# rewaifu/resselt

Measured on AMD Instinct MI355X. Metric: output megapixels/sec, RealESRGAN-x4plus 1080p→4K, 1/2/4/8 MI355X, higher is better.
Workload: dtype fp16; 1 GPU; RealESRGAN-x4plus (RRDBNet nf64 nb23 gc32 x4), 1x3x1080x1920 fp32 frame per GPU -> 1x3x4320x7680, residual-dense-block convolutions (92 % of the MACs) in ONE fp16 product on hi planes, conv_first / upsampling / HR / last convolutions in three bf16 products on split planes, trunk convolution in three fp16 products; f32 accumulate, synthetic uniform(+-1/sqrt(fan_in)) weights; precision=auto -> mixed, io=fp32 [N,C,H,W] tensors in and out, tile_parallel=single tile

## Files before the change

resselt_amd/csrc/conv_ring.h:

```cpp
#pragma once
#include <hip/hip_runtime.h>
#include <stdint.h>

#include "conv_common.h"
#include "conv_kernel.h"

namespace rsa {

#ifdef RSA_RING_DEBUG
static __device__ unsigned int g_ring_dbg;
#define RING_DBG(bit) (dbg & (bit))
#else
#define RING_DBG(bit) false
#endif

static __device__ unsigned int g_ring_aborts;

static unsigned int ring_aborts_this_unit() {
  unsigned int v = 0;
  const unsigned int zero = 0;
  if (hipMemcpyFromSymbol(&v, HIP_SYMBOL(g_ring_aborts), sizeof(v)) != hipSuccess) return 0x10000000u;
  if (v != 0 && hipMemcpyToSymbol(HIP_SYMBOL(g_ring_aborts), &zero, sizeof(zero)) != hipSuccess) return 0x10000000u;
  return v;
}

typedef const __attribute__((address_space(1))) char* gcptr;

#ifndef RSA_RING_INFL1
#define RSA_RING_INFL1 2
#endif
#ifndef RSA_RING_WD1
#define RSA_RING_WD1 3
#endif
#ifndef RSA_RING_WDX
#define RSA_RING_WDX 4
#endif
#ifndef RSA_RING_DEPTH1
#define RSA_RING_DEPTH1 4
#endif

template <int PROD, int WL = 0>
struct RingGeoP {
  static constexpr int TH = 16, TW = 32, IH = 18, IW = 34;
  static constexpr int PS = 624;
  static constexpr int HALF = 2 * PS;
  static constexpr int NHL = PROD == 3 ? 2 : 1;
  static constexpr int SLOT = NHL * HALF;
  static constexpr int NSLOT = (PROD == 3 || WL) ? 4 : 8;
  static constexpr int DMA_IT = (HALF + 63) / 64;
  static constexpr int DPF = NHL * DMA_IT;
  static constexpr int INFL = (PROD == 3 || WL) ? 1 : RSA_RING_INFL1;
  static constexpr int WL_FRAGS = WL ? 45 : 0;
  static constexpr int BAND = 4;
  static constexpr int FLAG_UNITS = 5;
};
using RingGeo = RingGeoP<3>;

__device__ __forceinline__ void ring_tile_coords(int t, int tiles_x, int tiles_y, int& n, int& ty, int& tx) {
  const int tiles_img = tiles_x * tiles_y;
  n = t / tiles_img;
  const int r = t - n * tiles_img;
  const int band = r / (RingGeo::BAND * tiles_x);
  const int rr = r - band * RingGeo::BAND * tiles_x;
  const int rows = min(RingGeo::BAND, tiles_y - band * RingGeo::BAND);
  tx = rr / rows;
  ty = band * RingGeo::BAND + (rr - tx * rows);
}

__device__ __forceinline__ uint32_t lds_ld(const uint32_t* p) { return __hip_atomic_load(p, __ATOMIC_RELAXED, __HIP_MEMORY_SCOPE_WORKGROUP); }

__device__ __forceinline__ void ring_wait_slow(const uint32_t* flag, uint32_t need, uint32_t* abort_word, const RingAux& aux) {
  const int limit = __builtin_amdgcn_readfirstlane(aux.spin_limit);
  for (int spin = 0; spin < limit; ++spin) {
    __builtin_amdgcn_s_sleep(1);
    if (__builtin_amdgcn_readfirstlane(lds_ld(flag)) >= need) return;
    if ((spin & 63) == 63 && __builtin_amdgcn_readfirstlane(lds_ld(abort_word)) != 0) return;
  }
  __hip_atomic_store(abort_word, 1u, __ATOMIC_RELAXED, __HIP_MEMORY_SCOPE_WORKGROUP);
  if ((threadIdx.x & 63) == 0) {
    atomicAdd(&g_ring_aborts, 1u);
    if (aux.fail_word != nullptr) __hip_atomic_fetch_add(aux.fail_word, 1u, __ATOMIC_RELAXED, __HIP_MEMORY_SCOPE_SYSTEM);
  }
}
__device__ __forceinline__ void ring_wait(const uint32_t* flag, uint32_t need, uint32_t* abort_word, const RingAux& aux) {
  if (__builtin_expect(__builtin_amdgcn_readfirstlane(lds_ld(flag)) < need, 0)) ring_wait_slow(flag, need, abort_word, aux);
}

__device__ __forceinline__ gcptr uniform_ptr(gcptr q) {
  const uint64_t v = (uint64_t)q;
  const uint32_t lo = __builtin_amdgcn_readfirstlane((uint32_t)v), hi = __builtin_amdgcn_readfirstlane((uint32_t)(v >> 32));
  return (gcptr)(((uint64_t)hi << 32) | lo);
}

__device__ __forceinline__ void dma16_s(uint32_t lds_addr, uint32_t voff, gcptr sbase) {
  asm volatile("s_mov_b32 m0, %0\n\ts_nop 0\n\tglobal_load_lds_dwordx4 %1, %2" ::"s"(lds_addr), "v"(voff), "s"(sbase) : "memory");
}
__device__ __forceinline__ void dma16_v(uint32_t lds_addr, gcptr vaddr) {
  asm volatile("s_mov_b32 m0, %0\n\ts_nop 0\n\tglobal_load_lds_dwordx4 %1, off" ::"s"(lds_addr), "v"(vaddr) : "memory");
}

#ifndef RSA_C5_EPI
#define RSA_C5_EPI 1
#endif
#ifdef RSA_C5_STAMPS
static __device__ unsigned long long g_c5_stamps[256 * 8 * 8];
#define C5_ST_ARG , st
#else
#define C5_ST_ARG
#endif
template <int SHAPE, int UP, int OUTK, int HM = 0, int FMT = 0, int PROD = 3, int XRES = 0, int XAC = 0, int XR2 = -1>
__global__ __launch_bounds__((8 + (SHAPE == 2 ? 2 : 1)) * 64, 3) void conv_ring(const rsa_conv_params p, const RingAux aux) {
  static_assert(XR2 == -1 || XRES == 4 || XRES == 5, "XR2: the coded conv5 kernels only");
  static_assert((XRES != 1 && XRES != 4 && XRES != 5) || (SHAPE == 1 && PROD == 1 && HM == 0 && UP == 0 && OUTK == 0), "XRES 1 / 4 / 5: conv5 of a residual dense block only");
  static_assert(XRES != 2 || (PROD == 1 && FMT == RSA_PF_F16 && OUTK == 0), "XRES 2: one fp16 product, hi-only plane output");
  static_assert(XRES != 3 || (SHAPE == 3 && PROD == 1 && FMT == RSA_PF_F16 && HM == 1 && UP == 0 && OUTK == 0), "XRES 3: the 48-channel SPAN-family layers");
  static_assert(XRES != 6 || (SHAPE == 2 && OUTK == 1 && UP == 0), "XRES 6: final stores with at most 16 output channels");
  static_assert(XRES != 7 || (SHAPE != 2 && UP == 0 && OUTK == 0), "XRES 7: plane output, one tile stream");
  constexpr bool WL = XRES == 3;
  constexpr bool XR = XRES == 1 || XRES == 4 || XRES == 5;
  using R = RingGeoP<PROD, WL>;
  constexpr int STREAMS = SHAPE == 2 ? 2 : 1;
  constexpr int TH = R::TH, TW = R::TW, IH = R::IH, IW = R::IW, PS = R::PS, HALF = R::HALF, SLOT = R::SLOT, NSLOT = R::NSLOT;
  constexpr int NHL = R::NHL, INFL = R::INFL;
  constexpr int WBASE = NSLOT * SLOT + R::FLAG_UNITS;
  constexpr int NCT = SHAPE == 2 ? 2 : (SHAPE == 1 ? 4 : 3);
  constexpr int CTW = SHAPE == 3 ? 3 : 2;
  constexpr int NPT = SHAPE == 3 ? 4 : 8;
  constexpr int CTU = XRES == 6 ? 1 : CTW;
  constexpr int RPW = NPT / 2;
  constexpr int NCONS = (STREAMS == 2) ? 4 : 8;
  constexpr int SPS = NSLOT / STREAMS;

  __shared__ uint4 s_ring[NSLOT * SLOT + R::FLAG_UNITS + R::WL_FRAGS * 64];
  uint32_t* const flags = (uint32_t*)&s_ring[NSLOT * SLOT];
  uint32_t* const f_full = flags;
  uint32_t* const f_free = flags + 8;
  uint32_t* const f_abort = flags + 16;

  const int tid = threadIdx.x;
  const int lane = tid & 63;
  const int wave = __builtin_amdgcn_readfirstlane(tid >> 6);

  const int tiles_x = (p.W + TW - 1) / TW;
  const int tiles_y = (p.H + TH - 1) / TH;
  const int num_tiles = tiles_x * tiles_y * p.batch;
  const int nhalf = p.cin_planes >> 1;
  const int nq = HM ? nhalf : (nhalf >> 1);
  const int ct_total = (p.cout + 15) >> 4;

  const int NWG = (int)gridDim.x;
  const int tile0 = (NWG % 8 == 0) ? ((int)blockIdx.x % 8) * (NWG / 8) + (int)blockIdx.x / 8 : (int)blockIdx.x;
  if (tile0 >= num_tiles) return;
  const int ntw = (num_tiles - tile0 + NWG - 1) / NWG;

  if (tid < 4 * R::FLAG_UNITS) flags[tid] = 0;
  if (WL) {
    const int wunits = nq * 5 * ct_total * 64;
    for (int i = tid; i < wunits; i += (int)blockDim.x) s_ring[WBASE + i] = ((const uint4*)p.w_packed)[i];
  }
  __syncthreads();
#ifdef RSA_RING_DEBUG
  const unsigned dbg = __builtin_amdgcn_readfirstlane(g_ring_dbg);
#endif

  if (wave >= 8) {
    __builtin_amdgcn_s_setprio(3);
    const int g = wave - 8;
    const int inW = UP ? (p.W >> 1) : p.W;
    uint32_t lc[R::DMA_IT];
    uint32_t smap[R::DMA_IT];
#pragma unroll
    for (int it = 0; it < R::DMA_IT; ++it) {
      const int u = it * 64 + lane;
      const int pl = (u / PS) & 1;
      const int r = u % PS;
      int py = r / IW, px = r - (r / IW) * IW;
      if (r >= IH * IW) py = 0, px = 0;
      smap[it] = (uint32_t)(pl << 16 | py << 8 | px);
      const int sy = UP ? ((py + 1) >> 1) : py;
      const int sx = UP ? ((px + 1) >> 1) : px;
      lc[it] = (uint32_t)(((int64_t)pl * p.in_plane_stride + (int64_t)sy * inW + sx) * 16);
    }
    const uint32_t ring_lds = (uint32_t)(uintptr_t)(__attribute__((address_space(3))) void*)s_ring;
    int k = 0;
    int pend_slot[INFL];
    uint32_t pend_val[INFL];
#pragma unroll
    for (int i = 0; i < INFL; ++i) pend_slot[i] = -1, pend_val[i] = 0;
    auto publish_all = [&]() {
      asm volatile("s_waitcnt vmcnt(0)" ::: "memory");
#pragma unroll
      for (int i = 0; i < INFL; ++i) {
        if (pend_slot[i] >= 0) __hip_atomic_store(&f_full[pend_slot[i]], pend_val[i], __ATOMIC_RELAXED, __HIP_MEMORY_SCOPE_WORKGROUP);
        pend_slot[i] = -1;
      }
    };
    for (int j = (STREAMS == 2 ? g : 0); j < ntw; j += STREAMS) {
      int n, ty, tx;
      ring_tile_coords(p.tile_order ? num_tiles - 1 - (tile0 + j * NWG) : tile0 + j * NWG, tiles_x, tiles_y, n, ty, tx);
      const int y0 = ty * TH - 1, x0 = tx * TW - 1;
      const bool interior = y0 >= 0 && x0 >= 0 && y0 + IH <= p.H && x0 + IW <= p.W;
      const int64_t tile_unit = (int64_t)n * p.in_batch_stride + (int64_t)(UP ? ty * (TH / 2) - 1 : y0) * inW + (UP ? tx * (TW / 2) - 1 : x0);
      for (int h = 0; h < nhalf; ++h, ++k) {
        const int slot = (STREAMS == 2) ? SPS * g + (k & (SPS - 1)) : (k & (NSLOT - 1));
        const uint32_t use = (uint32_t)(k / SPS);
        if (__builtin_amdgcn_readfirstlane(lds_ld(&f_free[slot])) < NCONS * use) {
          bool any = false;
#pragma unroll
          for (int i = 0; i < INFL; ++i) any = any || pend_slot[i] >= 0;
          if (any) publish_all();
          ring_wait(&f_free[slot], NCONS * use, f_abort, aux);
        }
        const int hh = XR ? 2 * (nq - 1 - (h >> 1)) + (h & 1) : h;
        const int64_t half_unit = tile_unit + (int64_t)(2 * hh) * p.in_plane_stride;
        gcptr bh = uniform_ptr((gcptr)p.in_hi + half_unit * 16);
        gcptr bl = uniform_ptr((gcptr)p.in_lo + half_unit * 16);
        const uint32_t dst = __builtin_amdgcn_readfirstlane(ring_lds + (uint32_t)slot * (SLOT * 16));
        if (RING_DBG(1)) {
        } else if (interior) {
#pragma unroll
          for (int it = 0; it < R::DMA_IT; ++it) {
            if (it == R::DMA_IT - 1 && lane >= 32) continue;
            dma16_s(dst + it * 1024, lc[it], bh);
            if (PROD == 3) dma16_s(dst + HALF * 16 + it * 1024, lc[it], bl);
          }
        } else {
#pragma unroll
          for (int it = 0; it < R::DMA_IT; ++it) {
            if (it == R::DMA_IT - 1 && lane >= 32) continue;
            const uint32_t m = smap[it];
            const int pl = (int)(m >> 16);
            int iy = y0 + (int)((m >> 8) & 255u), ix = x0 + (int)(m & 255u);
            const bool ok = (uint32_t)iy < (uint32_t)p.H && (uint32_t)ix < (uint32_t)p.W;
            if (UP) {
              iy >>= 1;
              ix >>= 1;
            }
            const int64_t off = ((int64_t)n * p.in_batch_stride + (int64_t)(2 * hh + pl) * p.in_plane_stride + (int64_t)iy * inW + ix) * 16;
            gcptr sh = ok ? (gcptr)p.in_hi + off : (gcptr)&g_zero_unit[0];
            dma16_v(dst + it * 1024, sh);
            if (PROD == 3) {
              gcptr sl = ok ? (gcptr)p.in_lo + off : (gcptr)&g_zero_unit[0];
              dma16_v(dst + HALF * 16 + it * 1024, sl);
            }
          }
        }
        if (pend_slot[0] >= 0) {
          asm volatile("s_waitcnt vmcnt(%0)" ::"n"(INFL * R::DPF) : "memory");
          __hip_atomic_store(&f_full[pend_slot[0]], pend_val[0], __ATOMIC_RELAXED, __HIP_MEMORY_SCOPE_WORKGROUP);
        }
#pragma unroll
        for (int i = 0; i + 1 < INFL; ++i) pend_slot[i] = pend_slot[i + 1], pend_val[i] = pend_val[i + 1];
        pend_slot[INFL - 1] = slot;
        pend_val[INFL - 1] = use + 1;
      }
    }
    publish_all();
    return;
  }

  const int g = (STREAMS == 2) ? (wave >> 2) : 0;
  const int wct = (SHAPE == 1) ? (wave >> 2) : 0;
  const int wpx = (SHAPE == 3) ? wave : (wave & 3);
  const int li = lane & 15;
  const int lg = lane >> 4;
  const int hsel = lg >> 1;

  constexpr int KSU = HM ? 5 : 9;
  constexpr int WD = (PROD == 3 || WL) ? 1 : ((XRES && XRES != 7) ? RSA_RING_WDX : RSA_RING_WD1);
  const int nks = nq * KSU;
  const __amdgpu_buffer_rsrc_t rw = __builtin_amdgcn_make_buffer_rsrc((void*)p.w_packed, 0, (uint32_t)((int64_t)nks * ct_total * NHL * 64 * 16), 0x00020000);
  uint32_t woff[CTW];
#pragma unroll
  for (int c = 0; c < CTW; ++c) {
    const int ctg = wct * CTW + c;
    woff[c] = (ctg < ct_total) ? (uint32_t)((ctg * NHL * 64 + lane) * 16) : 0xFFFFFFFFu;
  }
  const uint32_t wstep = (uint32_t)ct_total * NHL * 64 * 16;
  bf16x8 wq[WD + 1][CTW][NHL];
  auto load_w = [&](int s) {
#pragma unroll
    for (int c = 0; c < CTU; ++c)
#pragma unroll
      for (int hl = 0; hl < NHL; ++hl) {
        if (RING_DBG(4)) continue;
        if (WL) {
          wq[WD][c][hl] = *(const bf16x8*)&s_ring[WBASE + (s * ct_total + wct * CTW + c) * 64 + lane];
          continue;
        }
        const u32x4 v = __builtin_amdgcn_raw_buffer_load_b128(rw, woff[c], (uint32_t)s * wstep + (uint32_t)hl * 1024u, 0);
        wq[WD][c][hl] = __builtin_bit_cast(bf16x8, v);
      }
  };
  auto shift_w = [&]() {
#pragma unroll
    for (int d = 0; d < WD; ++d)
#pragma unroll
      for (int c = 0; c < CTU; ++c)
#pragma unroll
        for (int hl = 0; hl < NHL; ++hl) wq[d][c][hl] = wq[d + 1][c][hl];
  };

  f32x4 acc[NPT][CTW];
#pragma unroll
  for (int pt = 0; pt < NPT; ++pt)
#pragma unroll
    for (int ct = 0; ct < CTW; ++ct) acc[pt][ct] = (f32x4){0.f, 0.f, 0.f, 0.f};

  const int lane_u = (lg & 1) * PS + (wpx * RPW) * IW + li;
  int uA1, uA2, uB1, uB2, uS;

#ifndef RSA_RING_STAGGER
#define RSA_RING_STAGGER 0
#endif
#ifndef RSA_RING_STAGGER_SLEEP
#define RSA_RING_STAGGER_SLEEP 100
#endif
#ifndef RSA_RING_PRIO_HI
#define RSA_RING_PRIO_HI 0
#endif
  if (RSA_RING_PRIO_HI && wave >= 4) __builtin_amdgcn_s_setprio(RSA_RING_PRIO_HI);
  if (RSA_RING_STAGGER) {
    if (STREAMS == 2 ? g == 1 : wave >= 4)
      for (int d = 0; d < nq * RSA_RING_STAGGER; ++d) __builtin_amdgcn_s_sleep(RSA_RING_STAGGER_SLEEP);
  }

  auto wmap = [&](int c, int koff) -> int {
    int cc = c + koff / KSU;
    if (cc >= nq) cc -= nq;
    return (XR ? nq - 1 - cc : cc) * KSU + koff % KSU;
  };
#pragma unroll
  for (int d = 0; d < WD; ++d) {
    load_w(d < nks ? wmap(0, d) : wmap(0, 0));
    if (d + 1 < WD) {
#pragma unroll
      for (int e = 1; e < WD; ++e)
#pragma unroll
        for (int c = 0; c < CTW; ++c)
#pragma unroll
          for (int hl = 0; hl < NHL; ++hl) wq[e][c][hl] = wq[e + 1][c][hl];
    }
  }
  uint32_t kc = 0;
  auto slot_of = [&](uint32_t k) -> int { return (STREAMS == 2) ? SPS * g + (int)(k & (SPS - 1)) : (int)(k & (NSLOT - 1)); };
  auto use_of = [&](uint32_t k) -> uint32_t { return k / SPS; };
  uint32_t xslots = 0;
#ifdef RSA_C5_STAMPS
  unsigned long long st[8] = {0, 0, 0, 0, 0, 0, 0, 0};
  const unsigned long long t_begin = C5_TIME();
#endif
  for (int j = (STREAMS == 2 ? g : 0); j < ntw; j += STREAMS) {
    for (int c = 0; c < nq; ++c) {
      const int sA = slot_of(kc), sB = HM ? sA : slot_of(kc + 1);
      const uint32_t needA = use_of(kc) + 1, needB = use_of(kc + 1) + 1;
      if (XR) {
        if (c == nq - 2) xslots = (uint32_t)sA << 8 | (uint32_t)sB << 12;
        if (c == nq - 1) xslots |= (uint32_t)sA | (uint32_t)sB << 4;
      }
      {
        const int bA = sA * SLOT + lane_u, bB = sB * SLOT + lane_u;
        uA1 = bA + hsel;
        uA2 = bA + 2 + hsel * IW;
        uB1 = bB + hsel;
        uB2 = bB + 2 + hsel * IW;
        uS = (hsel ? bB : bA) + 2 * IW + 2;
      }
#ifdef RSA_C5_STAMPS
      const unsigned long long twA = C5_TIME();
#endif
      ring_wait(&f_full[sA], needA, f_abort, aux);
#ifdef RSA_C5_STAMPS
      st[1] += C5_TIME() - twA;
#endif
      __builtin_amdgcn_sched_barrier(0);
      asm volatile("" ::: "memory");

      constexpr int NSTEP = KSU * NPT;
      constexpr int DEPTH = PROD == 3 ? 2 : RSA_RING_DEPTH1;
      bf16x8 rh[DEPTH + 1], rl[PROD == 3 ? DEPTH + 1 : 1];
      auto frag = [&](int i) -> int {
        const int ks = i / NPT, pt = i % NPT;
        const int ptoff = (pt >> 1) * IW + (pt & 1) * 16;
        switch (ks) {
          case 0: return uA1 + ptoff;
          case 1: return uA1 + IW + ptoff;
          case 2: return uA1 + 2 * IW + ptoff;
          case 3: return uA2 + ptoff;
          case 4: return uS + ptoff;
          case 5: return uB1 + ptoff;
          case 6: return uB1 + IW + ptoff;
          case 7: return uB1 + 2 * IW + ptoff;
          default: return uB2 + ptoff;
        }
      };
#pragma unroll
      for (int i = 0; i < DEPTH; ++i) {
        rh[i] = *(const bf16x8*)&s_ring[frag(i)];
        if (PROD == 3) rl[i] = *(const bf16x8*)&s_ring[HALF + frag(i)];
      }
      auto step = [&](int i) {
        const int ks = i / NPT, sp = i % NPT;
        if (sp == 0) {
          shift_w();
          load_w(wmap(c, ks + WD));
          if (ks == 5) {
            asm volatile("" ::: "memory");
            if (lane == 0 && !(XR && c >= nq - 2)) __hip_atomic_fetch_add(&f_free[sA], 1u, __ATOMIC_RELAXED, __HIP_MEMORY_SCOPE_WORKGROUP);
          }
          __builtin_amdgcn_sched_barrier(0);
        }
        if (i + DEPTH < NSTEP && !RING_DBG(16)) {
          const int u = frag(i + DEPTH);
          rh[(i + DEPTH) % (DEPTH + 1)] = *(const bf16x8*)&s_ring[u];
          if (PROD == 3) rl[(i + DEPTH) % (DEPTH + 1)] = *(const bf16x8*)&s_ring[HALF + u];
        }
        if (!RING_DBG(2))
#pragma unroll
        for (int pr = 0; pr < PROD; ++pr)
#pragma unroll
          for (int ct = 0; ct < CTU; ++ct) {
            const bf16x8 wf = (PROD == 3 && pr == 0) ? wq[0][ct][NHL - 1] : wq[0][ct][0];
            const bf16x8 bf = (PROD == 3 && pr == 1) ? rl[PROD == 3 ? i % (DEPTH + 1) : 0] : rh[i % (DEPTH + 1)];
            acc[sp][ct] = mfma16<FMT>(wf, bf, acc[sp][ct]);
          }
        if (i + DEPTH < NSTEP) __builtin_amdgcn_sched_group_barrier(0x100, NHL, 0);
        __builtin_amdgcn_sched_group_barrier(0x008, PROD * CTU, 0);
        __builtin_amdgcn_sched_barrier(0);
      };
      if (HM) {
#pragma unroll
        for (int i = 0; i < NSTEP; ++i) step(i);
        asm volatile("" ::: "memory");
        if (lane == 0) __hip_atomic_fetch_add(&f_free[sA], 1u, __ATOMIC_RELAXED, __HIP_MEMORY_SCOPE_WORKGROUP);
        kc += 1;
      } else {
        constexpr int FIRST_B = 4 * NPT - DEPTH;
#pragma unroll
        for (int i = 0; i < FIRST_B; ++i) step(i);
#ifdef RSA_C5_STAMPS
        const unsigned long long twB = C5_TIME();
#endif
        ring_wait(&f_full[sB], needB, f_abort, aux);
#ifdef RSA_C5_STAMPS
        st[1] += C5_TIME() - twB;
#endif
        __builtin_amdgcn_sched_barrier(0);
        asm volatile("" ::: "memory");
#pragma unroll
        for (int i = FIRST_B; i < NSTEP; ++i) step(i);
        asm volatile("" ::: "memory");
        if (lane == 0 && !(XR && c >= nq - 2)) __hip_atomic_fetch_add(&f_free[sB], 1u, __ATOMIC_RELAXED, __HIP_MEMORY_SCOPE_WORKGROUP);
        kc += 2;
      }
    }
    {
      int n, ty, tx;
      ring_tile_coords(p.tile_order ? num_tiles - 1 - (tile0 + j * NWG) : tile0 + j * NWG, tiles_x, tiles_y, n, ty, tx);
      if (XRES == 2) {
        if (!RING_DBG(8)) epilogue_impl<NCT, CTW, NPT, 0, AC_LINEAR, 1, RSA_PF_F16>(p, acc, n, ty * TH, tx * TW, 0, wct, wpx, li, lg);
      } else if (XRES == 3) {
        if (!RING_DBG(8)) epilogue_impl<NCT, CTW, NPT, 0, XAC, 4, RSA_PF_F16>(p, acc, n, ty * TH, tx * TW, 0, wct, wpx, li, lg);
      } else if constexpr (XRES == 7) {
        if (!RING_DBG(8)) epilogue_impl<NCT, CTW, NPT, 0, AC_LINEAR, 5>(p, acc, n, ty * TH, tx * TW, 0, wct, wpx, li, lg);
      } else if (XR) {
#ifdef RSA_C5_STAMPS
        const unsigned long long te = C5_TIME();
#endif
        if (RING_DBG(8)) {
        } else if constexpr (XR2 >= 0) {
          epilogue_c5<XR2, XRES == 4 ? 1 : 2>(p, acc, n, ty * TH, tx * TW, wct, wpx, li, lg, s_ring, xslots, SLOT, PS, IW C5_ST_ARG);
        } else {
          if (p.res2_hi != nullptr)
            epilogue_impl<NCT, CTW, NPT, 0, AC_LINEAR, 3, RSA_PF_F16, 1, XRES == 4 ? 1 : (XRES == 5 ? 2 : 0)>(p, acc, n, ty * TH, tx * TW, 0, wct, wpx, li, lg, s_ring, xslots, SLOT, PS, IW C5_ST_ARG);
          else
            epilogue_impl<NCT, CTW, NPT, 0, AC_LINEAR, 2, RSA_PF_F16, 1, XRES == 4 ? 1 : (XRES == 5 ? 2 : 0)>(p, acc, n, ty * TH, tx * TW, 0, wct, wpx, li, lg, s_ring, xslots, SLOT, PS, IW C5_ST_ARG);
        }
#ifdef RSA_C5_STAMPS
        st[3] += C5_TIME() - te;
        st[4] += 1;
#endif
        asm volatile("s_waitcnt lgkmcnt(0)" ::: "memory");
        if (lane == 0) {
#pragma unroll
          for (int q = 0; q < 4; ++q) __hip_atomic_fetch_add(&f_free[(xslots >> (4 * q)) & 15u], 1u, __ATOMIC_RELAXED, __HIP_MEMORY_SCOPE_WORKGROUP);
        }
      } else if (!RING_DBG(8)) {
        epilogue<NCT, CTW, NPT, OUTK>(p, acc, n, ty * TH, tx * TW, 0, wct, wpx, li, lg);
      }
    }
#pragma unroll
    for (int pt = 0; pt < NPT; ++pt)
#pragma unroll
      for (int ct = 0; ct < CTW; ++ct) acc[pt][ct] = (f32x4){0.f, 0.f, 0.f, 0.f};
  }
#ifdef RSA_C5_STAMPS
  st[0] = C5_TIME() - t_begin;
  if (XR && lane == 0 && blockIdx.x < 256)
    for (int i = 0; i < 8; ++i) g_c5_stamps[((int)blockIdx.x * 8 + wave) * 8 + i] = st[i];
#endif
}

template <int SHAPE, int UP, int OUTK, int HM = 0, int FMT = 0, int PROD = 3, int XRES = 0, int XAC = 0, int XR2 = -1>
static int launch_ring(const rsa_conv_params& p, hipStream_t stream) {
  if constexpr ((XRES == 4 || XRES == 5) && XR2 == -1 && RSA_C5_EPI) {
    if (c5_epilogue_fits(p))
      return p.res2_hi != nullptr ? launch_ring<SHAPE, UP, OUTK, HM, FMT, PROD, XRES, XAC, 1>(p, stream) : launch_ring<SHAPE, UP, OUTK, HM, FMT, PROD, XRES, XAC, 0>(p, stream);
  }
  constexpr int STREAMS = SHAPE == 2 ? 2 : 1;
  using R = RingGeoP<PROD>;
  const int tiles_x = (p.W + R::TW - 1) / R::TW;
  const int tiles_y = (p.H + R::TH - 1) / R::TH;
  const int64_t num_tiles = (int64_t)tiles_x * tiles_y * p.batch;
  if (num_tiles > 0x3fffffff) return RSA_E_UNSUPPORTED;
  static const int cus = [] {
    int dev = 0;
    hipDeviceProp_t prop;
    if (hipGetDevice(&dev) != hipSuccess || hipGetDeviceProperties(&prop, dev) != hipSuccess) return 256;
    return prop.multiProcessorCount;
  }();
  int gx = cus;
  if (gx > num_tiles) gx = (int)num_tiles;
  hipLaunchKernelGGL((conv_ring<SHAPE, UP, OUTK, HM, FMT, PROD, XRES, XAC, XR2>), dim3((unsigned)gx, 1, 1), dim3((8 + STREAMS) * 64), 0, stream, p, ring_aux());
  return (int)hipGetLastError();
}

}
```

resselt_amd/csrc/conv_ring_pair.h:

```cpp
#pragma once
#include <type_traits>

#include "conv_ring.h"

namespace rsa {

struct PairParams {
  int32_t batch, H, W;
  int32_t nqa;
  const void* in_hi;
  int64_t in_plane_stride, in_batch_stride;
  const void* wa;
  const void* wb;
  const float* bias_a;
  const float* bias_b;
  float slope_a, slope_b;
  void* outa_hi;
  int64_t outa_unit0;
  int64_t outa_plane_stride, outa_batch_stride;
  void* outb_hi;
  int64_t outb_unit0;
  int64_t outb_plane_stride, outb_batch_stride;
  int32_t tile_order;
};

#ifndef RSA_PAIR_INFL
#define RSA_PAIR_INFL 1
#endif
#ifndef RSA_PAIR_WD
#define RSA_PAIR_WD 3
#endif
#ifndef RSA_PAIR_DEPTH
#define RSA_PAIR_DEPTH 3
#endif
#ifndef RSA_PAIR_PRIO_B
#define RSA_PAIR_PRIO_B 1
#endif
#ifndef RSA_PAIR_PRIO_A
#define RSA_PAIR_PRIO_A 0
#endif

#ifdef RSA_PAIR_STAMPS
static __device__ unsigned long long g_pair_stamps[256 * 9 * 8];
#define PSTAMP() __builtin_amdgcn_s_memtime()
#define PST_ADD(slot, t0) st[slot] += PSTAMP() - (t0)
#else
#define PSTAMP() 0ull
#define PST_ADD(slot, t0) (void)(t0)
#endif

struct PairGeo {
  static constexpr int TH = 16, TWO = 30;
  static constexpr int AH = 18, AW = 32;
  static constexpr int IH = 20, IW = 34;
  static constexpr int PS = 688;
  static constexpr int SLOT = 2 * PS;
  static constexpr int NSLOT = 5;
  static constexpr int DMA_IT = (SLOT + 63) / 64;
  static constexpr int INFL = RSA_PAIR_INFL;
  static constexpr int PSB = AH * AW;
  static constexpr int XB0 = NSLOT * SLOT;
  static constexpr int XB_UNITS = 4 * PSB + 16;
  static constexpr int FLAG_UNITS = 4;
  static constexpr int LDS_UNITS = XB0 + XB_UNITS + FLAG_UNITS;
  static_assert(SLOT % 64 == 32, "the last LDS-DMA instruction of a fill covers 32 units");
  static_assert(INFL * DMA_IT <= 63, "vmcnt");
  static_assert(LDS_UNITS * 16 <= 160 * 1024, "LDS");
};

__device__ __forceinline__ uint32_t pack_f16(float a, float b) {
  const f16x2 h = {(_Float16)a, (_Float16)b};
  return __builtin_bit_cast(uint32_t, h);
}

__device__ __forceinline__ uint4 pair_unit_f16(const f32x4 a, const f32x4 b, const f32x4 bias, float slope) {
  float va[4], vb[4];
#pragma unroll
  for (int r = 0; r < 4; ++r) {
    va[r] = a[r] + bias[r];
    vb[r] = b[r] + bias[r];
    va[r] = fmaxf(va[r], va[r] * slope);
    vb[r] = fmaxf(vb[r], vb[r] * slope);
  }
  const uint32_t a0 = pack_f16(va[0], va[1]), a1 = pack_f16(va[2], va[3]);
  const uint32_t b0 = pack_f16(vb[0], vb[1]), b1 = pack_f16(vb[2], vb[3]);
  const u32x2 h0 = __builtin_amdgcn_permlane16_swap(a0, b0, false, false);
  const u32x2 h1 = __builtin_amdgcn_permlane16_swap(a1, b1, false, false);
  return make_uint4(h0.x, h1.x, h0.y, h1.y);
}

template <int ROLE>
__device__ __forceinline__ void pair_consumer(const PairParams& p, const RingAux& aux, uint4* s_ring, uint32_t* flags, int wave, int lane, int tile0, int ntw,
                                              int NWG, int tiles_x, int tiles_y, int num_tiles) {
  using G = PairGeo;
  constexpr int IW = G::IW, PS = G::PS, SLOT = G::SLOT, NSLOT = G::NSLOT, AW = G::AW, PSB = G::PSB, XB0 = G::XB0;
  constexpr int CTW = 2, KSU = 9;
  constexpr int WD = RSA_PAIR_WD, DEPTH = RSA_PAIR_DEPTH;
  constexpr bool roleB = ROLE == 1;
  constexpr int NPT = roleB ? 8 : 9;
  uint32_t* const f_full = flags;
  uint32_t* const f_free = flags + 5;
  uint32_t* const f_abort = flags + 10;
  uint32_t* const f_xfull = flags + 11;
  uint32_t* const f_xfree = flags + 12;
  const int nqa = p.nqa;
#ifdef RSA_RING_DEBUG
  const unsigned dbg = __builtin_amdgcn_readfirstlane(g_ring_dbg);
#endif
  if (roleB && RSA_PAIR_PRIO_B) __builtin_amdgcn_s_setprio(RSA_PAIR_PRIO_B);
  if (!roleB && RSA_PAIR_PRIO_A) __builtin_amdgcn_s_setprio(RSA_PAIR_PRIO_A);
  const int r4 = wave & 3;
  const int li = lane & 15;
  const int lg = lane >> 4;
  const int hsel = lg >> 1;

  const int nunits = roleB ? nqa + 1 : nqa;
  const int nks = nunits * KSU;
  const __amdgpu_buffer_rsrc_t rw = __builtin_amdgcn_make_buffer_rsrc((void*)(roleB ? p.wb : p.wa), 0, (uint32_t)(nks * CTW * 64 * 16), 0x00020000);
  uint32_t woff[CTW];
#pragma unroll
  for (int c = 0; c < CTW; ++c) woff[c] = (uint32_t)((c * 64 + lane) * 16);
  constexpr uint32_t wstep = CTW * 64 * 16;
  bf16x8 wq[WD + 1][CTW];
  auto load_w = [&](int s) {
#pragma unroll
    for (int c = 0; c < CTW; ++c) {
      if (RING_DBG(4)) continue;
      const u32x4 v = __builtin_amdgcn_raw_buffer_load_b128(rw, woff[c], (uint32_t)s * wstep, 0);
      wq[WD][c] = __builtin_bit_cast(bf16x8, v);
    }
  };
  auto shift_w = [&]() {
#pragma unroll
    for (int d = 0; d < WD; ++d)
#pragma unroll
      for (int c = 0; c < CTW; ++c) wq[d][c] = wq[d + 1][c];
  };
  auto wmap = [&](int c, int koff) -> int {
    int cc = c + koff / KSU;
    if (cc >= nunits) cc -= nunits;
    return cc * KSU + koff % KSU;
  };
#pragma unroll
  for (int d = 0; d < WD; ++d) {
    load_w(d < nks ? wmap(0, d) : wmap(0, 0));
    if (d + 1 < WD) {
#pragma unroll
      for (int e = 1; e < WD; ++e)
#pragma unroll
        for (int c = 0; c < CTW; ++c) wq[e][c] = wq[e + 1][c];
    }
  }

  f32x4 acc[NPT][CTW];
#pragma unroll
  for (int pt = 0; pt < NPT; ++pt)
#pragma unroll
    for (int ct = 0; ct < CTW; ++ct) acc[pt][ct] = (f32x4){0.f, 0.f, 0.f, 0.f};

  const int lane_u = (lg & 1) * PS + (4 * r4 + (roleB ? 1 : 0)) * IW + li + (roleB ? 1 : 0);
  const int extra_u = __builtin_amdgcn_readfirstlane((16 + (r4 >> 1) - 4 * r4) * IW + (r4 & 1) * 16);
  const int lane_ub = XB0 + (lg & 1) * PSB + (4 * r4) * AW + li;

  int slot = 0;
  uint32_t use = 0;
  uint32_t tcount = 0;
#ifdef RSA_PAIR_STAMPS
  unsigned long long st[8] = {0, 0, 0, 0, 0, 0, 0, 0};
  const unsigned long long t_begin = PSTAMP();
#endif

  auto run_unit = [&](auto rs_tag, auto ring_tag, int c, int bA, int bB, int sA, int sB, uint32_t needA, uint32_t needB) {
    constexpr int RS = decltype(rs_tag)::value;
    constexpr bool RING = decltype(ring_tag)::value;
    constexpr int NSTEP = KSU * NPT;
    const int uA1 = bA + hsel, uA2 = bA + 2 + hsel * RS, uB1 = bB + hsel, uB2 = bB + 2 + hsel * RS;
    const int uS = (hsel ? bB : bA) + 2 * RS + 2;
    {
      const unsigned long long tw = PSTAMP();
      if (RING) ring_wait(&f_full[sA], needA, f_abort, aux);
      if (RING) PST_ADD(1, tw);
    }
    __builtin_amdgcn_sched_barrier(0);
    asm volatile("" ::: "memory");
    bf16x8 rh[DEPTH + 1];
    auto frag = [&](int i) -> int {
      const int ks = i / NPT, pt = i % NPT;
      const int ptoff = pt < 8 ? (pt >> 1) * RS + (pt & 1) * 16 : extra_u;
      switch (ks) {
        case 0: return uA1 + ptoff;
        case 1: return uA1 + RS + ptoff;
        case 2: return uA1 + 2 * RS + ptoff;
        case 3: return uA2 + ptoff;
        case 4: return uS + ptoff;
        case 5: return uB1 + ptoff;
        case 6: return uB1 + RS + ptoff;
        case 7: return uB1 + 2 * RS + ptoff;
        default: return uB2 + ptoff;
      }
    };
#pragma unroll
    for (int i = 0; i < DEPTH; ++i) rh[i] = *(const bf16x8*)&s_ring[frag(i)];
    auto step = [&](int i) {
      const int ks = i / NPT, sp = i % NPT;
      if (sp == 0) {
        shift_w();
        load_w(wmap(c, ks + WD));
        if (RING && ks == 5) {
          asm volatile("" ::: "memory");
          if (lane == 0) __hip_atomic_fetch_add(&f_free[sA], 1u, __ATOMIC_RELAXED, __HIP_MEMORY_SCOPE_WORKGROUP);
        }
        __builtin_amdgcn_sched_barrier(0);
      }
      if (i + DEPTH < NSTEP && !RING_DBG(16)) rh[(i + DEPTH) % (DEPTH + 1)] = *(const bf16x8*)&s_ring[frag(i + DEPTH)];
      if (!RING_DBG(2))
#pragma unroll
      for (int ct = 0; ct < CTW; ++ct) acc[sp][ct] = mfma16<RSA_PF_F16>(wq[0][ct], rh[i % (DEPTH + 1)], acc[sp][ct]);
      if (i + DEPTH < NSTEP) __builtin_amdgcn_sched_group_barrier(0x100, 1, 0);
      __builtin_amdgcn_sched_group_barrier(0x008, CTW, 0);
      __builtin_amdgcn_sched_barrier(0);
    };
    constexpr int FIRST_B = 4 * NPT - DEPTH;
#pragma unroll
    for (int i = 0; i < FIRST_B; ++i) step(i);
    {
      const unsigned long long tw = PSTAMP();
      if (RING) ring_wait(&f_full[sB], needB, f_abort, aux);
      if (RING) PST_ADD(1, tw);
    }
    __builtin_amdgcn_sched_barrier(0);
    asm volatile("" ::: "memory");
#pragma unroll
    for (int i = FIRST_B; i < NSTEP; ++i) step(i);
    asm volatile("" ::: "memory");
    if (RING && lane == 0) __hip_atomic_fetch_add(&f_free[sB], 1u, __ATOMIC_RELAXED, __HIP_MEMORY_SCOPE_WORKGROUP);
  };
  using std::integral_constant;

  for (int j = 0; j < ntw; ++j) {
    for (int c = 0; c < nqa; ++c) {
      const int sA = slot;
      const uint32_t needA = use + 1;
      if (++slot == NSLOT) slot = 0, ++use;
      const int sB = slot;
      const uint32_t needB = use + 1;
      if (++slot == NSLOT) slot = 0, ++use;
      run_unit(integral_constant<int, IW>{}, integral_constant<bool, true>{}, c, sA * SLOT + lane_u, sB * SLOT + lane_u, sA, sB, needA, needB);
    }
    int n, ty, tx;
    ring_tile_coords(p.tile_order ? num_tiles - 1 - (tile0 + j * NWG) : tile0 + j * NWG, tiles_x, tiles_y, n, ty, tx);
    const int y0 = ty * G::TH, x0 = tx * G::TWO;
    int lli = li, llg = lg;
    asm volatile("" : "+v"(lli), "+v"(llg));
    const int plane_l = llg >> 1;
    const int col = 16 * (llg & 1) + lli;
    if (!roleB) {
      const unsigned long long tx0 = PSTAMP();
      ring_wait(f_xfree, 4u * tcount, f_abort, aux);
      PST_ADD(2, tx0);
      const unsigned long long te0 = PSTAMP();
      char* const ob = (char*)p.outa_hi + (p.outa_unit0 + (int64_t)n * p.outa_batch_stride + (int64_t)(y0 - 1) * p.W + (x0 - 1)) * 16;
      const int x = x0 - 1 + col;
      const bool xin = (uint32_t)x < (uint32_t)p.W;
      const bool xst = xin && col >= 1 && col <= G::TWO;
#pragma unroll
      for (int ct = 0; ct < CTW; ++ct) {
        if (RING_DBG(8)) break;
        const f32x4 bias = p.bias_a != nullptr ? ((const f32x4*)p.bias_a)[ct * 4 + llg] : (f32x4){0.f, 0.f, 0.f, 0.f};
        const uint32_t pl_off = (uint32_t)(2 * ct + plane_l);
#pragma unroll
        for (int pp = 0; pp < 4; ++pp) {
          uint4 u = pair_unit_f16(acc[2 * pp][ct], acc[2 * pp + 1][ct], bias, p.slope_a);
          const int ra = 4 * r4 + pp;
          const int y = y0 - 1 + ra;
          const bool yin = (uint32_t)y < (uint32_t)p.H;
          if (!(yin && xin)) u = make_uint4(0u, 0u, 0u, 0u);
          s_ring[XB0 + pl_off * PSB + ra * AW + col] = u;
          if (yin && xst && ra >= 1) *(uint4*)(ob + (pl_off * (uint32_t)p.outa_plane_stride + (uint32_t)(ra * p.W + col)) * 16u) = u;
          __builtin_amdgcn_sched_barrier(0);
        }
        {
          uint4 u = pair_unit_f16(acc[NPT - 1][ct], acc[NPT - 1][ct], bias, p.slope_a);
          const int ra = 16 + (r4 >> 1);
          const int ecol = 16 * (r4 & 1) + lli;
          const int y = y0 - 1 + ra, xe = x0 - 1 + ecol;
          const bool yin = (uint32_t)y < (uint32_t)p.H, xein = (uint32_t)xe < (uint32_t)p.W;
          if (!(yin && xein)) u = make_uint4(0u, 0u, 0u, 0u);
          if ((llg & 1) == 0) {
            s_ring[XB0 + pl_off * PSB + ra * AW + ecol] = u;
            if (yin && xein && ra <= 16 && ecol >= 1 && ecol <= G::TWO)
              *(uint4*)(ob + (pl_off * (uint32_t)p.outa_plane_stride + (uint32_t)(ra * p.W + ecol)) * 16u) = u;
          }
          __builtin_amdgcn_sched_barrier(0);
        }
      }
      asm volatile("s_waitcnt lgkmcnt(0)" ::: "memory");
      if (lane == 0) __hip_atomic_fetch_add(f_xfull, 1u, __ATOMIC_RELAXED, __HIP_MEMORY_SCOPE_WORKGROUP);
      PST_ADD(3, te0);
    } else {
      const unsigned long long tx0 = PSTAMP();
      ring_wait(f_xfull, 4u * (tcount + 1u), f_abort, aux);
      PST_ADD(2, tx0);
      const unsigned long long tu0 = PSTAMP();
      if (!RING_DBG(32)) run_unit(integral_constant<int, AW>{}, integral_constant<bool, false>{}, nqa, lane_ub, lane_ub + 2 * PSB, 0, 0, 0u, 0u);
      if (lane == 0) __hip_atomic_fetch_add(f_xfree, 1u, __ATOMIC_RELAXED, __HIP_MEMORY_SCOPE_WORKGROUP);
      PST_ADD(4, tu0);
      const unsigned long long te0 = PSTAMP();
      char* const ob = (char*)p.outb_hi + (p.outb_unit0 + (int64_t)n * p.outb_batch_stride + (int64_t)y0 * p.W + x0) * 16;
      const bool xst = x0 + col < p.W && col < G::TWO;
#pragma unroll
      for (int ct = 0; ct < CTW; ++ct) {
        if (RING_DBG(8)) break;
        const f32x4 bias = p.bias_b != nullptr ? ((const f32x4*)p.bias_b)[ct * 4 + llg] : (f32x4){0.f, 0.f, 0.f, 0.f};
        const uint32_t pl_off = (uint32_t)(2 * ct + plane_l);
#pragma unroll
        for (int pp = 0; pp < 4; ++pp) {
          const uint4 u = pair_unit_f16(acc[2 * pp][ct], acc[2 * pp + 1][ct], bias, p.slope_b);
          const int rb = 4 * r4 + pp;
          if (y0 + rb < p.H && xst) *(uint4*)(ob + (pl_off * (uint32_t)p.outb_plane_stride + (uint32_t)(rb * p.W + col)) * 16u) = u;
          __builtin_amdgcn_sched_barrier(0);
        }
      }
      PST_ADD(3, te0);
    }
#pragma unroll
    for (int pt = 0; pt < NPT; ++pt)
#pragma unroll
      for (int ct = 0; ct < CTW; ++ct) acc[pt][ct] = (f32x4){0.f, 0.f, 0.f, 0.f};
    ++tcount;
  }
#ifdef RSA_PAIR_STAMPS
  st[0] = PSTAMP() - t_begin;
  st[5] = tcount;
  if (lane == 0 && blockIdx.x < 256)
    for (int i = 0; i < 8; ++i) g_pair_stamps[((int)blockIdx.x * 9 + wave) * 8 + i] = st[i];
#endif
}


__global__ __launch_bounds__(9 * 64, 3) void conv_ring_pair(const PairParams p, const RingAux aux) {
  using G = PairGeo;
  constexpr int IW = G::IW, PS = G::PS, SLOT = G::SLOT, NSLOT = G::NSLOT, AW = G::AW, PSB = G::PSB, XB0 = G::XB0, INFL = G::INFL;
  constexpr int NCONS = 8;
  constexpr int CTW = 2, KSU = 9;
  constexpr int WD = RSA_PAIR_WD, DEPTH = RSA_PAIR_DEPTH;

  __shared__ uint4 s_ring[G::LDS_UNITS];
  uint32_t* const flags = (uint32_t*)&s_ring[XB0 + G::XB_UNITS];
  uint32_t* const f_full = flags;
  uint32_t* const f_free = flags + 5;
  uint32_t* const f_abort = flags + 10;
  uint32_t* const f_xfull = flags + 11;
  uint32_t* const f_xfree = flags + 12;

  const int tid = threadIdx.x;
  const int lane = tid & 63;
  const int wave = __builtin_amdgcn_readfirstlane(tid >> 6);

  const int tiles_x = (p.W + G::TWO - 1) / G::TWO;
  const int tiles_y = (p.H + G::TH - 1) / G::TH;
  const int num_tiles = tiles_x * tiles_y * p.batch;
  const int nqa = p.nqa;
  const int nhalf = 2 * nqa;

  const int NWG = (int)gridDim.x;
  const int tile0 = (NWG % 8 == 0) ? ((int)blockIdx.x % 8) * (NWG / 8) + (int)blockIdx.x / 8 : (int)blockIdx.x;
  if (tile0 >= num_tiles) return;
  const int ntw = (num_tiles - tile0 + NWG - 1) / NWG;

  if (tid < 4 * G::FLAG_UNITS) flags[tid] = 0;
  __syncthreads();
#ifdef RSA_RING_DEBUG
  const unsigned dbg = __builtin_amdgcn_readfirstlane(g_ring_dbg);
#endif

  if (wave == 8) {
    __builtin_amdgcn_s_setprio(3);
    uint32_t lc[G::DMA_IT];
    uint32_t smap[G::DMA_IT];
#pragma unroll
    for (int it = 0; it < G::DMA_IT; ++it) {
      const int u = it * 64 + lane;
      const int pl = (u / PS) & 1;
      const int r = u % PS;
      int py = r / IW, px = r - (r / IW) * IW;
      if (r >= G::IH * IW) py = 0, px = 0;
      smap[it] = (uint32_t)(pl << 16 | py << 8 | px);
      lc[it] = (uint32_t)(((int64_t)pl * p.in_plane_stride + (int64_t)py * p.W + px) * 16);
    }
    const uint32_t ring_lds = (uint32_t)(uintptr_t)(__attribute__((address_space(3))) void*)s_ring;
    int slot = 0;
    uint32_t use = 0;
    int pend_slot[INFL];
    uint32_t pend_val[INFL];
#pragma unroll
    for (int i = 0; i < INFL; ++i) pend_slot[i] = -1, pend_val[i] = 0;
    auto publish_all = [&]() {
      asm volatile("s_waitcnt vmcnt(0)" ::: "memory");
#pragma unroll
      for (int i = 0; i < INFL; ++i) {
        if (pend_slot[i] >= 0) __hip_atomic_store(&f_full[pend_slot[i]], pend_val[i], __ATOMIC_RELAXED, __HIP_MEMORY_SCOPE_WORKGROUP);
        pend_slot[i] = -1;
      }
    };
#ifdef RSA_PAIR_STAMPS
    unsigned long long st[8] = {0, 0, 0, 0, 0, 0, 0, 0};
    const unsigned long long t_begin = PSTAMP();
#endif
    for (int j = 0; j < ntw; ++j) {
      int n, ty, tx;
      ring_tile_coords(p.tile_order ? num_tiles - 1 - (tile0 + j * NWG) : tile0 + j * NWG, tiles_x, tiles_y, n, ty, tx);
      const int y0 = ty * G::TH - 2, x0 = tx * G::TWO - 2;
      const bool interior = y0 >= 0 && x0 >= 0 && y0 + G::IH <= p.H && x0 + IW <= p.W;
      const int64_t tile_unit = (int64_t)n * p.in_batch_stride + (int64_t)y0 * p.W + x0;
      for (int h = 0; h < nhalf; ++h) {
        if (__builtin_amdgcn_readfirstlane(lds_ld(&f_free[slot])) < NCONS * use) {
          bool any = false;
#pragma unroll
          for (int i = 0; i < INFL; ++i) any = any || pend_slot[i] >= 0;
          const unsigned long long tw = PSTAMP();
          if (any) publish_all();
          ring_wait(&f_free[slot], NCONS * use, f_abort, aux);
          PST_ADD(1, tw);
        }
        const int64_t half_unit = tile_unit + (int64_t)(2 * h) * p.in_plane_stride;
        gcptr bh = uniform_ptr((gcptr)p.in_hi + half_unit * 16);
        const uint32_t dst = __builtin_amdgcn_readfirstlane(ring_lds + (uint32_t)slot * (SLOT * 16));
        if (RING_DBG(1)) {
        } else if (interior) {
#pragma unroll
          for (int it = 0; it < G::DMA_IT; ++it) {
            if (it == G::DMA_IT - 1 && lane >= 32) continue;
            dma16_s(dst + it * 1024, lc[it], bh);
          }
        } else {
#pragma unroll
          for (int it = 0; it < G::DMA_IT; ++it) {
            if (it == G::DMA_IT - 1 && lane >= 32) continue;
            const uint32_t m = smap[it];
            const int pl = (int)(m >> 16);
            const int iy = y0 + (int)((m >> 8) & 255u), ix = x0 + (int)(m & 255u);
            const bool ok = (uint32_t)iy < (uint32_t)p.H && (uint32_t)ix < (uint32_t)p.W;
            const int64_t off = ((int64_t)n * p.in_batch_stride + (int64_t)(2 * h + pl) * p.in_plane_stride + (int64_t)iy * p.W + ix) * 16;
            gcptr sh = ok ? (gcptr)p.in_hi + off : (gcptr)&g_zero_unit[0];
            dma16_v(dst + it * 1024, sh);
          }
        }
        if (pend_slot[0] >= 0) {
          const unsigned long long tw = PSTAMP();
          asm volatile("s_waitcnt vmcnt(%0)" ::"n"(INFL * G::DMA_IT) : "memory");
          PST_ADD(2, tw);
          __hip_atomic_store(&f_full[pend_slot[0]], pend_val[0], __ATOMIC_RELAXED, __HIP_MEMORY_SCOPE_WORKGROUP);
        }
#pragma unroll
        for (int i = 0; i + 1 < INFL; ++i) pend_slot[i] = pend_slot[i + 1], pend_val[i] = pend_val[i + 1];
        pend_slot[INFL - 1] = slot;
        pend_val[INFL - 1] = use + 1;
        if (++slot == NSLOT) slot = 0, ++use;
      }
    }
    publish_all();
#ifdef RSA_PAIR_STAMPS
    st[0] = PSTAMP() - t_begin;
    if (lane == 0 && blockIdx.x < 256)
      for (int i = 0; i < 8; ++i) g_pair_stamps[((int)blockIdx.x * 9 + 8) * 8 + i] = st[i];
#endif
    return;
  }

  if (wave >= 4)
    pair_consumer<1>(p, aux, s_ring, flags, wave, lane, tile0, ntw, NWG, tiles_x, tiles_y, num_tiles);
  else
    pair_consumer<0>(p, aux, s_ring, flags, wave, lane, tile0, ntw, NWG, tiles_x, tiles_y, num_tiles);
}

}
```

Measured before the change: 382.8 output megapixels/s.

## Reuse each LDS row fragment across three vertical kernel taps via row sweep

Adds a RowSweep schedule for the 3x3 convolution ring consumers, in both the single-product ring kernel and the paired kernel. Each loaded input row fragment feeds the MFMAs of up to three output rows, one per kernel row tap, instead of being reloaded once per tap. The aim is fewer LDS reads per MFMA in the dense-block convolutions. In exchange the weight registers have to be rotated across taps (wq indexed by dy), which raises register pressure and makes the schedule and the slot-free signalling more complex.

```diff
diff --git a/resselt_amd/csrc/conv_ring.h b/resselt_amd/csrc/conv_ring.h
--- a/resselt_amd/csrc/conv_ring.h
+++ b/resselt_amd/csrc/conv_ring.h
@@ -38,6 +38,44 @@
 #ifndef RSA_RING_DEPTH1
 #define RSA_RING_DEPTH1 4
 #endif
+
+#ifndef RSA_RING_ROWSWEEP
+#define RSA_RING_ROWSWEEP 3
+#endif
+
+template <int RPW, int NPT>
+struct RowSweep {
+  static constexpr int NX = NPT - 2 * RPW;
+  static constexpr int SW = 2 * (RPW + 2) + 3 * NX;
+  static constexpr int F3 = SW, F4 = F3 + NPT, F5 = F4 + NPT, F8 = F5 + SW, NF = F8 + NPT;
+  struct Step {
+    int k0;
+    int q;
+    int ir, hf;
+    int xdy;
+    int shifts;
+    bool sweep, rotate;
+  };
+  static constexpr Step at(int f) {
+    Step s{};
+    s.sweep = f < F3 || (f >= F5 && f < F8);
+    s.k0 = f < F3 ? 0 : f < F4 ? 3 : f < F5 ? 4 : f < F8 ? 5 : 8;
+    s.q = f < F3 ? f : f < F4 ? f - F3 : f < F5 ? f - F4 : f < F8 ? f - F5 : f - F8;
+    s.ir = -1;
+    if (s.sweep) {
+      if (s.q >= 2 * RPW && s.q < 2 * RPW + 3 * NX) {
+        s.xdy = s.q - 2 * RPW;
+      } else {
+        const int qq = s.q < 2 * RPW ? s.q : s.q - 3 * NX;
+        s.ir = qq >> 1;
+        s.hf = qq & 1;
+        s.shifts = s.ir >= RPW ? s.ir - RPW + 1 : 0;
+      }
+    }
+    s.rotate = s.q == 0 || (s.sweep && s.ir >= RPW && s.hf == 0);
+    return s;
+  }
+};
 
 template <int PROD, int WL = 0>
 struct RingGeoP {
@@ -378,6 +416,7 @@
 
       constexpr int NSTEP = KSU * NPT;
       constexpr int DEPTH = PROD == 3 ? 2 : RSA_RING_DEPTH1;
+      constexpr bool SWEEP = (RSA_RING_ROWSWEEP & 1) && PROD == 1 && !HM && SHAPE != 3 && WD >= 2;
       bf16x8 rh[DEPTH + 1], rl[PROD == 3 ? DEPTH + 1 : 1];
       auto frag = [&](int i) -> int {
         const int ks = i / NPT, pt = i % NPT;
@@ -428,7 +467,63 @@
         __builtin_amdgcn_sched_group_barrier(0x008, PROD * CTU, 0);
         __builtin_amdgcn_sched_barrier(0);
       };
-      if (HM) {
+      if constexpr (SWEEP) {
+        using RS = RowSweep<RPW, NPT>;
+        static_assert(DEPTH <= NPT && DEPTH <= RS::SW, "the prologue reads the first fragments of K step 0 / of the half-A sweep");
+        auto sfrag = [&](int f) -> int {
+          const auto s = RS::at(f);
+          return (s.k0 == 0 ? uA1 : s.k0 == 3 ? uA2 : s.k0 == 4 ? uS : s.k0 == 5 ? uB1 : uB2) + (s.q >> 1) * IW + (s.q & 1) * 16;
+        };
+        auto sstep = [&](int f) {
+          const auto s = RS::at(f);
+          if (s.rotate) {
+            shift_w();
+            load_w(wmap(c, s.k0 + s.shifts + WD));
+            if (f == RS::F5) {
+              asm volatile("" ::: "memory");
+              if (lane == 0 && !(XR && c >= nq - 2)) __hip_atomic_fetch_add(&f_free[sA], 1u, __ATOMIC_RELAXED, __HIP_MEMORY_SCOPE_WORKGROUP);
+            }
+            __builtin_amdgcn_sched_barrier(0);
+          }
+          if (f + DEPTH < RS::NF && !RING_DBG(16)) rh[(f + DEPTH) % (DEPTH + 1)] = *(const bf16x8*)&s_ring[sfrag(f + DEPTH)];
+          if (f + DEPTH < RS::NF) __builtin_amdgcn_sched_group_barrier(0x100, 1, 0);
+          const bf16x8 bf = rh[f % (DEPTH + 1)];
+          if (s.sweep) {
+#pragma unroll
+            for (int dy = 0; dy < 3; ++dy) {
+              const int r = s.ir - dy;
+              if (r < 0 || r >= RPW) continue;
+              if (!RING_DBG(2))
+#pragma unroll
+                for (int ct = 0; ct < CTU; ++ct) acc[2 * r + s.hf][ct] = mfma16<FMT>(wq[dy - s.shifts][ct][0], bf, acc[2 * r + s.hf][ct]);
+            }
+            __builtin_amdgcn_sched_group_barrier(0x008, 3 * CTU, 0);
+          } else {
+            if (!RING_DBG(2))
+#pragma unroll
+              for (int ct = 0; ct < CTU; ++ct) acc[s.q][ct] = mfma16<FMT>(wq[0][ct][0], bf, acc[s.q][ct]);
+            __builtin_amdgcn_sched_group_barrier(0x008, CTU, 0);
+          }
+          __builtin_amdgcn_sched_barrier(0);
+        };
+        constexpr int FIRST_B = RS::F4 - DEPTH;
+#pragma unroll
+        for (int f = 0; f < FIRST_B; ++f) sstep(f);
+#ifdef RSA_C5_STAMPS
+        const unsigned long long twB = C5_TIME();
+#endif
+        ring_wait(&f_full[sB], needB, f_abort, aux);
+#ifdef RSA_C5_STAMPS
+        st[1] += C5_TIME() - twB;
+#endif
+        __builtin_amdgcn_sched_barrier(0);
+        asm volatile("" ::: "memory");
+#pragma unroll
+        for (int f = FIRST_B; f < RS::NF; ++f) sstep(f);
+        asm volatile("" ::: "memory");
+        if (lane == 0 && !(XR && c >= nq - 2)) __hip_atomic_fetch_add(&f_free[sB], 1u, __ATOMIC_RELAXED, __HIP_MEMORY_SCOPE_WORKGROUP);
+        kc += 2;
+      } else if (HM) {
 #pragma unroll
         for (int i = 0; i < NSTEP; ++i) step(i);
         asm volatile("" ::: "memory");
diff --git a/resselt_amd/csrc/conv_ring_pair.h b/resselt_amd/csrc/conv_ring_pair.h
--- a/resselt_amd/csrc/conv_ring_pair.h
+++ b/resselt_amd/csrc/conv_ring_pair.h
@@ -98,6 +98,7 @@
   constexpr int WD = RSA_PAIR_WD, DEPTH = RSA_PAIR_DEPTH;
   constexpr bool roleB = ROLE == 1;
   constexpr int NPT = roleB ? 8 : 9;
+  constexpr bool SWEEP = (RSA_RING_ROWSWEEP & 2) && WD >= 2;
   uint32_t* const f_full = flags;
   uint32_t* const f_free = flags + 5;
   uint32_t* const f_abort = flags + 10;
@@ -220,20 +221,78 @@
       __builtin_amdgcn_sched_group_barrier(0x008, CTW, 0);
       __builtin_amdgcn_sched_barrier(0);
     };
-    constexpr int FIRST_B = 4 * NPT - DEPTH;
-#pragma unroll
-    for (int i = 0; i < FIRST_B; ++i) step(i);
-    {
-      const unsigned long long tw = PSTAMP();
-      if (RING) ring_wait(&f_full[sB], needB, f_abort, aux);
-      if (RING) PST_ADD(1, tw);
-    }
-    __builtin_amdgcn_sched_barrier(0);
-    asm volatile("" ::: "memory");
-#pragma unroll
-    for (int i = FIRST_B; i < NSTEP; ++i) step(i);
-    asm volatile("" ::: "memory");
-    if (RING && lane == 0) __hip_atomic_fetch_add(&f_free[sB], 1u, __ATOMIC_RELAXED, __HIP_MEMORY_SCOPE_WORKGROUP);
+    if constexpr (SWEEP) {
+      using SO = RowSweep<4, NPT>;
+      static_assert(DEPTH <= 8, "the prologue reads the first fragments of K step 0 / of the half-A sweep");
+      auto sfrag = [&](int f) -> int {
+        const auto s = SO::at(f);
+        const int base = s.k0 == 0 ? uA1 : s.k0 == 3 ? uA2 : s.k0 == 4 ? uS : s.k0 == 5 ? uB1 : uB2;
+        if (s.sweep) return base + (s.ir >= 0 ? s.ir * RS + s.hf * 16 : s.xdy * RS + extra_u);
+        return base + (s.q < 8 ? (s.q >> 1) * RS + (s.q & 1) * 16 : extra_u);
+      };
+      auto sstep = [&](int f) {
+        const auto s = SO::at(f);
+        if (s.rotate) {
+          shift_w();
+          load_w(wmap(c, s.k0 + s.shifts + WD));
+          if (RING && f == SO::F5) {
+            asm volatile("" ::: "memory");
+            if (lane == 0) __hip_atomic_fetch_add(&f_free[sA], 1u, __ATOMIC_RELAXED, __HIP_MEMORY_SCOPE_WORKGROUP);
+          }
+          __builtin_amdgcn_sched_barrier(0);
+        }
+        if (f + DEPTH < SO::NF && !RING_DBG(16)) rh[(f + DEPTH) % (DEPTH + 1)] = *(const bf16x8*)&s_ring[sfrag(f + DEPTH)];
+        if (f + DEPTH < SO::NF) __builtin_amdgcn_sched_group_barrier(0x100, 1, 0);
+        const bf16x8 bf = rh[f % (DEPTH + 1)];
+        if (s.sweep && s.ir >= 0) {
+#pragma unroll
+          for (int dy = 0; dy < 3; ++dy) {
+            const int r = s.ir - dy;
+            if (r < 0 || r >= 4) continue;
+            if (!RING_DBG(2))
+#pragma unroll
+              for (int ct = 0; ct < CTW; ++ct) acc[2 * r + s.hf][ct] = mfma16<RSA_PF_F16>(wq[dy - s.shifts][ct], bf, acc[2 * r + s.hf][ct]);
+            __builtin_amdgcn_sched_group_barrier(0x008, CTW, 0);
+          }
+        } else {
+          const int pt = s.sweep ? NPT - 1 : s.q, kw = s.sweep ? s.xdy : 0;
+          if (!RING_DBG(2))
+#pragma unroll
+            for (int ct = 0; ct < CTW; ++ct) acc[pt][ct] = mfma16<RSA_PF_F16>(wq[kw][ct], bf, acc[pt][ct]);
+          __builtin_amdgcn_sched_group_barrier(0x008, CTW, 0);
+        }
+        __builtin_amdgcn_sched_barrier(0);
+      };
+      constexpr int FIRST_B = SO::F4 - DEPTH;
+#pragma unroll
+      for (int f = 0; f < FIRST_B; ++f) sstep(f);
+      {
+        const unsigned long long tw = PSTAMP();
+        if (RING) ring_wait(&f_full[sB], needB, f_abort, aux);
+        if (RING) PST_ADD(1, tw);
+      }
+      __builtin_amdgcn_sched_barrier(0);
+      asm volatile("" ::: "memory");
+#pragma unroll
+      for (int f = FIRST_B; f < SO::NF; ++f) sstep(f);
+      asm volatile("" ::: "memory");
+      if (RING && lane == 0) __hip_atomic_fetch_add(&f_free[sB], 1u, __ATOMIC_RELAXED, __HIP_MEMORY_SCOPE_WORKGROUP);
+    } else {
+      constexpr int FIRST_B = 4 * NPT - DEPTH;
+#pragma unroll
+      for (int i = 0; i < FIRST_B; ++i) step(i);
+      {
+        const unsigned long long tw = PSTAMP();
+        if (RING) ring_wait(&f_full[sB], needB, f_abort, aux);
+        if (RING) PST_ADD(1, tw);
+      }
+      __builtin_amdgcn_sched_barrier(0);
+      asm volatile("" ::: "memory");
+#pragma unroll
+      for (int i = FIRST_B; i < NSTEP; ++i) step(i);
+      asm volatile("" ::: "memory");
+      if (RING && lane == 0) __hip_atomic_fetch_add(&f_free[sB], 1u, __ATOMIC_RELAXED, __HIP_MEMORY_SCOPE_WORKGROUP);
+    }
   };
   using std::integral_constant;
 
```

New measurement: 385.9 output megapixels/s (median of 6 runs). No clear change (+0.8%).
